# ecpoppenheimer/TensorFlowRayTrace

Measured on AMD Instinct MI355X. Metric: ray-surface intersection tests/sec (fwd+bwd), higher is better.
Workload: dtype f32 ray state, f32 filter + f64 decisions

## Files before the change

### tensorflowraytrace_amd/csrc/tfrt_trace3d.hip

```cpp
#include <vector>

#include <type_traits>
#include "tfrt_common.h"
#include "goal_finish.h"
#include "wave_schedule.h"

namespace tfrt {

constexpr int TILE = 512;
constexpr int KC = 24;

constexpr int ERR_CAPACITY = 1;


__global__ __launch_bounds__(BLOCK) void k_center(const double* __restrict__ fverts, int M,
                                                  double* __restrict__ c0, int32_t* nrays0, int n,
                                                  int32_t* tail8, unsigned int* scan_ticket) {
  if (nrays0 != nullptr) {
    if (threadIdx.x == 0) *nrays0 = n;
    if (threadIdx.x < 8) tail8[threadIdx.x] = 0;
    if (threadIdx.x == 0 && scan_ticket != nullptr) *scan_ticket = 0u;
  }
  __shared__ double red[WAVES][3];
  __shared__ double ctr[3];
// ... 1183 lines not shown
  float nx0, ny0, c0, nx1, ny1, c1, nx2, ny2, c2;
  edge(q0x, q0y, g1x, g1y, &nx0, &ny0, &c0);
  edge(q0x + g1x, q0y + g1y, g2x - g1x, g2y - g1y, &nx1, &ny1, &c1);
  edge(q0x + g2x, q0y + g2y, -g2x, -g2y, &nx2, &ny2, &c2);
  if (flat) {
    nx0 = ny0 = nx1 = ny1 = nx2 = ny2 = 0.f;
    c0 = c1 = c2 = -INFINITY;
  }
  const float slack2 = 1.5f * slack;
  rec[0] = make_float4(nx0, ny0, c0, tlo);
  rec[1] = make_float4(nx1, ny1, c1, thi);
  rec[2] = make_float4(nx2, ny2, c2, 0.5f * (tlo + thi));
  rec[3] = make_float4(0.5001f * (thi - tlo), slack2, r0.w, 0.f);
  const float rho = (fminf(b.R0 + b.S * fmaxf(fabsf(tlo), fabsf(thi)),
                           b.R0b + b.S * fmaxf(fabsf(tlo - b.tb), fabsf(thi - b.tb))) +
                     slack2) * 1.0001f;
  return !(c0 > rho) && !(c1 > rho) && !(c2 > rho) && !(thi < b.tmin);
}

template <typename Op>
__device__ __forceinline__ float wave_reduce_f(float v, Op op) {
  auto dpp = [](float x, auto ctrl, auto row_mask) {
    return __int_as_float(__builtin_amdgcn_update_dpp(__float_as_int(x), __float_as_int(x),
                                                      decltype(ctrl)::value,
                                                      decltype(row_mask)::value, 0xF, false));
  };
  using std::integral_constant;
  v = op(v, dpp(v, integral_constant<int, 0xB1>{}, integral_constant<int, 0xF>{}));
  v = op(v, dpp(v, integral_constant<int, 0x4E>{}, integral_constant<int, 0xF>{}));
  v = op(v, dpp(v, integral_constant<int, 0x141>{}, integral_constant<int, 0xF>{}));
  v = op(v, dpp(v, integral_constant<int, 0x140>{}, integral_constant<int, 0xF>{}));
  v = op(v, dpp(v, integral_constant<int, 0x142>{}, integral_constant<int, 0xA>{}));
  v = op(v, dpp(v, integral_constant<int, 0x143>{}, integral_constant<int, 0xC>{}));
  return __int_as_float(__builtin_amdgcn_readlane(__float_as_int(v), 63));
}
__device__ __forceinline__ float wave_sum_f(float v) {
  return wave_reduce_f(v, [](float a, float b) { return a + b; });
}
__device__ __forceinline__ float wave_max_f(float v) {
  return wave_reduce_f(v, [](float a, float b) { return fmaxf(a, b); });
}
__device__ __forceinline__ float wave_min_f(float v) {
  return wave_reduce_f(v, [](float a, float b) { return fminf(a, b); });
}
#define TFRT_DPP_STEP4(OPA, OPB, OPC, OPD, CTRL)      \
  OPA " %0, %0, %0 " CTRL "\n\t" OPB " %1, %1, %1 " CTRL "\n\t" \
  OPC " %2, %2, %2 " CTRL "\n\t" OPD " %3, %3, %3 " CTRL "\n\t"
#define TFRT_DPP_ALL4(OPA, OPB, OPC, OPD)                                        \
  "s_nop 1\n\t"                                                                  \
  TFRT_DPP_STEP4(OPA, OPB, OPC, OPD, "quad_perm:[1,0,3,2] row_mask:0xf bank_mask:0xf") \
  TFRT_DPP_STEP4(OPA, OPB, OPC, OPD, "quad_perm:[2,3,0,1] row_mask:0xf bank_mask:0xf") \
  TFRT_DPP_STEP4(OPA, OPB, OPC, OPD, "row_half_mirror row_mask:0xf bank_mask:0xf")     \
  TFRT_DPP_STEP4(OPA, OPB, OPC, OPD, "row_mirror row_mask:0xf bank_mask:0xf")          \
  TFRT_DPP_STEP4(OPA, OPB, OPC, OPD, "row_bcast:15 row_mask:0xa bank_mask:0xf")        \
  TFRT_DPP_STEP4(OPA, OPB, OPC, OPD, "row_bcast:31 row_mask:0xc bank_mask:0xf")
__device__ __forceinline__ void wave_sum4(float& a, float& b, float& c, float& d) {
  __asm__ volatile(TFRT_DPP_ALL4("v_add_f32_dpp", "v_add_f32_dpp", "v_add_f32_dpp", "v_add_f32_dpp")
                   : "+v"(a), "+v"(b), "+v"(c), "+v"(d));
  a = __int_as_float(__builtin_amdgcn_readlane(__float_as_int(a), 63));
  b = __int_as_float(__builtin_amdgcn_readlane(__float_as_int(b), 63));
  c = __int_as_float(__builtin_amdgcn_readlane(__float_as_int(c), 63));
  d = __int_as_float(__builtin_amdgcn_readlane(__float_as_int(d), 63));
}
__device__ __forceinline__ void wave_max3_min(float& a, float& b, float& c, float& d) {
  __asm__ volatile(TFRT_DPP_ALL4("v_max_f32_dpp", "v_max_f32_dpp", "v_max_f32_dpp", "v_min_f32_dpp")
                   : "+v"(a), "+v"(b), "+v"(c), "+v"(d));
  a = __int_as_float(__builtin_amdgcn_readlane(__float_as_int(a), 63));
  b = __int_as_float(__builtin_amdgcn_readlane(__float_as_int(b), 63));
  c = __int_as_float(__builtin_amdgcn_readlane(__float_as_int(c), 63));
  d = __int_as_float(__builtin_amdgcn_readlane(__float_as_int(d), 63));
}

#define TFRT_DPP_STEP3(OPA, OPB, OPC, CTRL) \
  OPA " %0, %0, %0 " CTRL "\n\t" OPB " %1, %1, %1 " CTRL "\n\t" OPC " %2, %2, %2 " CTRL "\n\t"
#define TFRT_DPP_ALL3(OPA, OPB, OPC)                                        \
  "s_nop 1\n\t"                                                             \
  TFRT_DPP_STEP3(OPA, OPB, OPC, "quad_perm:[1,0,3,2] row_mask:0xf bank_mask:0xf") \
  TFRT_DPP_STEP3(OPA, OPB, OPC, "quad_perm:[2,3,0,1] row_mask:0xf bank_mask:0xf") \
  TFRT_DPP_STEP3(OPA, OPB, OPC, "row_half_mirror row_mask:0xf bank_mask:0xf")     \
  TFRT_DPP_STEP3(OPA, OPB, OPC, "row_mirror row_mask:0xf bank_mask:0xf")          \
  TFRT_DPP_STEP3(OPA, OPB, OPC, "row_bcast:15 row_mask:0xa bank_mask:0xf")        \
  TFRT_DPP_STEP3(OPA, OPB, OPC, "row_bcast:31 row_mask:0xc bank_mask:0xf")
__device__ __forceinline__ void wave_sum2_max(float& a, float& b, float& c) {
  __asm__ volatile(TFRT_DPP_ALL3("v_add_f32_dpp", "v_add_f32_dpp", "v_max_f32_dpp")
                   : "+v"(a), "+v"(b), "+v"(c));
  a = __int_as_float(__builtin_amdgcn_readlane(__float_as_int(a), 63));
  b = __int_as_float(__builtin_amdgcn_readlane(__float_as_int(b), 63));
  c = __int_as_float(__builtin_amdgcn_readlane(__float_as_int(c), 63));
}

#define TFRT_BCAST(K) " row_newbcast:" #K " row_mask:0xf bank_mask:0xf\n\t"
__device__ __forceinline__ void face_edges(const float word, const float Ax, const float Ay,
                                           const float Mx, const float My, const float Mlen,
                                           const float Perr, const float Pm, float& room,
                                           float& e0, float& e1, float& e2) {
  float ix, iy;
  __asm__ volatile(
      "s_nop 1\n\t"
      "v_mov_b32_dpp %3, %6" TFRT_BCAST(11)
      "v_mov_b32_dpp %0, %6" TFRT_BCAST(13)
      "v_fma_f32 %5, %3, %10, %8\n\t"
      "v_fma_f32 %4, %3, %9, %7\n\t"
      "v_fmac_f32_dpp %0, %6, %11" TFRT_BCAST(12)
      "v_mul_f32_dpp %1, %6, %5" TFRT_BCAST(1)
      "v_mul_f32_dpp %2, %6, %5" TFRT_BCAST(5)
      "v_add_f32 %0, %12, %0\n\t"
      "v_fma_f32 %0, %13, |%3|, %0\n\t"
      "v_fmac_f32_dpp %1, %6, %4" TFRT_BCAST(0)
      "v_fmac_f32_dpp %2, %6, %4" TFRT_BCAST(4)
      "v_mul_f32_dpp %3, %6, %5" TFRT_BCAST(9)
      "v_add_f32_dpp %1, %6, %1" TFRT_BCAST(2)
      "v_add_f32_dpp %2, %6, %2" TFRT_BCAST(6)
      "v_fmac_f32_dpp %3, %6, %4" TFRT_BCAST(8)
      "s_nop 1\n\t"
      "v_add_f32_dpp %3, %6, %3" TFRT_BCAST(10)
      : "=&v"(room), "=&v"(e0), "=&v"(e1), "=&v"(e2), "=&v"(ix), "=&v"(iy)
      : "v"(word), "v"(Ax), "v"(Ay), "v"(Mx), "v"(My), "v"(Mlen), "v"(Perr), "v"(Pm));
}

__device__ __forceinline__ float uniform_f(float v) {
  return __int_as_float(__builtin_amdgcn_readfirstlane(__float_as_int(v)));
}
__device__ __forceinline__ float bcast_f(float v, int src_lane) {
  return __int_as_float(__builtin_amdgcn_readlane(__float_as_int(v), src_lane));
}

template <typename U>
using LdsPtr = __attribute__((address_space(3))) U*;

template <typename RT>
__device__ __forceinline__ void beam_decide(const int nb, const int lane, LdsPtr<const uint32_t> x_pair,
                                         LdsPtr<const RT> rt, LdsPtr<unsigned long long> best_k,
                                         LdsPtr<int32_t> best_i, const double* __restrict__ fverts,
                                         const double eps_int, const double eps_size,
                                         const double eps_start) {
  bool have = false;
  unsigned long long key = 0, old = 0;
  int j = -1;
  const uint32_t xp = lane < nb ? x_pair[lane] : 0u;
  const int slot = (int)(xp & 63u);
  if (lane < nb) {
    double s[3], e[3];
#pragma unroll
    for (int k = 0; k < 3; ++k) {
      s[k] = static_cast<double>(rt[k * 64 + slot]);
      e[k] = static_cast<double>(rt[(3 + k) * 64 + slot]);
    }
    j = (int)(xp >> 6);
    old = best_k[slot];
    double P[9];
    const double* fp = fverts + 9 * (int64_t)j;
#pragma unroll
    for (int k = 0; k < 9; ++k) P[k] = fp[k];
    const TriHit h = exact_triangle(s, e, P, eps_int, eps_size, eps_start);
    if (h.valid) {
      have = true;
      key = dkey(h.ray_u);
    }
  }
  wave_fence();
  if (have) atomicMin((unsigned long long*)&best_k[slot], key);
  wave_fence();
  bool win = false;
  if (have) {
    const unsigned long long now = best_k[slot];
    win = key == now;
    if (win && now < old) best_i[slot] = 0x7FFFFFFF;
  }
  wave_fence();
  if (win) atomicMin((int32_t*)&best_i[slot], j);
  wave_fence();
}

template <typename RT>
struct BeamLds {
  uint16_t slist[BEAM_SLIST];
  uint16_t clist[BEAM_CLIST];
  uint32_t flist[BEAM_FLIST];
  uint32_t x_pair[192];
  float4 ftab[65][4];
  RT rtab[6][64];
  unsigned long long best_k[64];
  int32_t best_i[64];
};

struct BeamScene {
  const float4* susphere;
  const float4* clsphere;
  const float4* csphere;
  const float4* crec;
  const double* fverts;
  const double* c0;
  int n_clusters, n_super;
  double eps_int, eps_size, eps_start;
};

#ifdef TFRT_TICKS
#define TFRT_WI_ARG _wi
#else
#define TFRT_WI_ARG nullptr
#endif

template <typename T, typename RT>
__device__ __forceinline__ bool beam_pass(BeamLds<RT>& W, const BeamScene& g, const int lane,
                                          const int bundle, const bool live, const int skip,
                                          const bool first_pass, const int coherent_only,
                                          unsigned* _wi, unsigned* work = nullptr) {
  TFRT_TICK_INIT;
  const float4* __restrict__ susphere = g.susphere;
  const float4* __restrict__ clsphere = g.clsphere;
  const float4* __restrict__ csphere = g.csphere;
  const float4* __restrict__ crec = g.crec;
  const double* __restrict__ fverts = g.fverts;
  const double* __restrict__ c0 = g.c0;
  const int n_clusters = g.n_clusters, n_super = g.n_super;
  const double eps_int = g.eps_int, eps_size = g.eps_size, eps_start = g.eps_start;
  const float4 never = make_float4(0.f, 0.f, 0.f, -1.f);
  W.best_k[lane] = dkey(INFINITY);
  W.best_i[lane] = -1;
  const double cx = c0[0], cy = c0[1], cz = c0[2];
  const float cxf = uniform_f((float)cx), cyf = uniform_f((float)cy), czf = uniform_f((float)cz);
  auto rel = [](const RT v, const double c, const float cf) -> float {
    if constexpr (sizeof(T) <= 4) return (float)v - cf;
    else return (float)((double)v - c);
  };
  const float es_f = (float)eps_size;
  int xn = 0;

  auto decide = [&](const int nb) {
    TFRT_STAT(28, 1);
    TFRT_WAVE_NOTE(1, 1);
    wave_fence();
    beam_decide<RT>(nb, lane, (LdsPtr<const uint32_t>)&W.x_pair[0],
                    (LdsPtr<const RT>)&W.rtab[0][0], (LdsPtr<unsigned long long>)&W.best_k[0],
                    (LdsPtr<int32_t>)&W.best_i[0], fverts, eps_int, eps_size, eps_start);
  };

  TFRT_STAT(8, 1);
  constexpr int BEAM_ATTEMPTS = 20;
  TFRT_TICK(0);
  float gap = -1.f;
  unsigned long long cuts = 0ull;
  int lo = 0, attempts = 0;
  bool spread = false;
  while (lo < bundle) {
    ++attempts;
    TFRT_STAT(30, 1);
    TFRT_WAVE_NOTE(0, 1);
    const unsigned long long above = lo < 63 ? (cuts >> (lo + 1)) << (lo + 1) : 0ull;
    const int hi = above != 0ull ? __ffsll((long long)above) - 1 : bundle;
    const int len = hi - lo;
    wave_fence();
    RT own[6];
#pragma unroll
    for (int k = 0; k < 6; ++k) own[k] = W.rtab[k][lane];
    const float sx = rel(own[0], cx, cxf), sy = rel(own[1], cy, cyf), sz = rel(own[2], cz, czf);
    const float dx = (float)(own[3] - own[0]), dy = (float)(own[4] - own[1]),
                dz = (float)(own[5] - own[2]);
    const float len2 = dx * dx + dy * dy + dz * dz;
    const bool ok = live && len2 > 0.f && len2 < 3.0e38f;
    const float inv = ok ? __builtin_amdgcn_rsqf(len2) : 0.f;
    const float ux = dx * inv, uy = dy * inv, uz = dz * inv;
    const float rabs = fabsf(sx) + fabsf(sy) + fabsf(sz);
    const bool sel = ok && lane >= lo && lane < hi;
    const float4 su_first = lane < n_super ? susphere[lane] : never;
    const float cnt = (float)__popcll(__ballot(sel));
    bool narrow = true, brute = false;
    int ns = 0, nc = 0, nf = 0;
    Beam bm = {0.f, 0.f, 0.f, 0.f, 0.f, 1.f, 0.f, 0.f, -INFINITY, 1.f, 0.f, 0.f, 0.f, 1.f, 0.f,
               INFINITY, 0.f};
    float ray_t = 0.f, ray_dt = 0.f, ray_terr = 0.f;
    float Ax = 0.f, Ay = 0.f, Mx = 0.f, My = 0.f, Mlen = 0.f, Perr = 0.f, Pm = 0.f;
    if (cnt > 0.f) {
      float swx = sel ? ux : 0.f, swy = sel ? uy : 0.f, swz = sel ? uz : 0.f;
      float sox = sel ? sx : 0.f, soy = sel ? sy : 0.f, soz = sel ? sz : 0.f;
      float Lw = sel ? rabs : 0.f;
      wave_sum4(swx, swy, swz, sox);
      wave_sum2_max(soy, soz, Lw);
      const float wl2 = swx * swx + swy * swy + swz * swz;
      narrow = wl2 > 0.49f * cnt * cnt;
      spread = !narrow;
      const float wi = narrow ? __builtin_amdgcn_rsqf(wl2) : 0.f;
      bm.wx = swx * wi; bm.wy = swy * wi; bm.wz = swz * wi;
      const float icnt = __builtin_amdgcn_rcpf(cnt);
      bm.ox = sox * icnt; bm.oy = soy * icnt; bm.oz = soz * icnt;
      const float cosk = ux * bm.wx + uy * bm.wy + uz * bm.wz;
      if (__any(sel && !(cosk > 0.7f))) narrow = false, spread = true;
      const float px = sx - bm.ox, py = sy - bm.oy, pz = sz - bm.oz;
      const float ts = px * bm.wx + py * bm.wy + pz * bm.wz;
      ray_t = ts;
      ray_dt = dx * bm.wx + dy * bm.wy + dz * bm.wz;
      ray_terr = 1e-5f * (rabs + fabsf(bm.ox) + fabsf(bm.oy) + fabsf(bm.oz));
      {
        const float f0 = fabsf(bm.wx), f1 = fabsf(bm.wy), f2 = fabsf(bm.wz);
        const bool k0 = f0 <= f1 && f0 <= f2, k1 = !k0 && f1 <= f2;
        const float kx = k0 ? 1.f : 0.f, ky = k1 ? 1.f : 0.f, kz = (!k0 && !k1) ? 1.f : 0.f;
        const float cxx = bm.wy * kz - bm.wz * ky, cyy = bm.wz * kx - bm.wx * kz,
                    czz = bm.wx * ky - bm.wy * kx;
        const float il = __builtin_amdgcn_rsqf(cxx * cxx + cyy * cyy + czz * czz);
        bm.e1x = cxx * il; bm.e1y = cyy * il; bm.e1z = czz * il;
        bm.e2x = bm.wy * bm.e1z - bm.wz * bm.e1y;
        bm.e2y = bm.wz * bm.e1x - bm.wx * bm.e1z;
        bm.e2z = bm.wx * bm.e1y - bm.wy * bm.e1x;
      }
      {
        const float idt = __builtin_amdgcn_rcpf(sel ? ray_dt : 1.f);
        Mx = (dx * bm.e1x + dy * bm.e1y + dz * bm.e1z) * idt;
        My = (dx * bm.e2x + dy * bm.e2y + dz * bm.e2z) * idt;
        const float p1 = px * bm.e1x + py * bm.e1y + pz * bm.e1z,
                    p2 = px * bm.e2x + py * bm.e2y + pz * bm.e2z;
        Ax = p1 - ts * Mx;
        Ay = p2 - ts * My;
        Mlen = __builtin_amdgcn_sqrtf(Mx * Mx + My * My) * 1.0001f;
        Pm = 2e-5f * (fabsf(Mx) + fabsf(My));
        Perr = 2e-5f * (fabsf(p1) + fabsf(p2) + fabsf(ts) * (fabsf(Mx) + fabsf(My)) + rabs +
                        fabsf(bm.ox) + fabsf(bm.oy) + fabsf(bm.oz));
      }
      float R0 = sel ? __builtin_amdgcn_sqrtf(Ax * Ax + Ay * Ay) : 0.f, S = sel ? Mlen : 0.f;
      float tmin = sel ? ts : INFINITY;
      Lw += fabsf(bm.ox) + fabsf(bm.oy) + fabsf(bm.oz);
      const float tb = -(bm.ox * bm.wx + bm.oy * bm.wy + bm.oz * bm.wz);
      float R0b = 0.f;
      if (sel) {
        const float bx = Ax + Mx * tb, by = Ay + My * tb;
        R0b = __builtin_amdgcn_sqrtf(bx * bx + by * by);
      }
      wave_max3_min(R0, S, R0b, tmin);
      bm.R0 = R0 * 1.001f + 4e-6f * Lw;
      bm.S = S * 1.001f + 2e-6f;
      bm.tb = tb;
      bm.R0b = R0b * 1.001f + 4e-6f * (Lw + fabsf(tb)) + 2e-6f * fabsf(tb) * S;
      if (!(bm.R0b < 3.0e38f)) bm.R0b = INFINITY;
      bm.tmin = (!first_pass && eps_start >= 0.0) ? tmin - 1e-5f * Lw - 1e-5f * fabsf(tmin)
                                                  : -INFINITY;
      if (!(bm.R0 < 3.0e38f && bm.S < 3.0e38f)) narrow = false;
      bm.ox = uniform_f(bm.ox); bm.oy = uniform_f(bm.oy); bm.oz = uniform_f(bm.oz);
      bm.wx = uniform_f(bm.wx); bm.wy = uniform_f(bm.wy); bm.wz = uniform_f(bm.wz);
      bm.R0 = uniform_f(bm.R0); bm.S = uniform_f(bm.S); bm.tmin = uniform_f(bm.tmin);
      bm.R0b = uniform_f(bm.R0b); bm.tb = uniform_f(bm.tb);
      bm.e1x = uniform_f(bm.e1x); bm.e1y = uniform_f(bm.e1y); bm.e1z = uniform_f(bm.e1z);
      bm.e2x = uniform_f(bm.e2x); bm.e2y = uniform_f(bm.e2y); bm.e2z = uniform_f(bm.e2z);
      TFRT_TICK(1);

      if (narrow) {
        float4 nxt = su_first;
        for (int b = 0; b < n_super; b += 64) {
          const int node = b + lane;
          const float4 cur = nxt;
          nxt = node + 64 < n_super ? susphere[node + 64] : never;
          const bool hit = beam_touch(bm, cur);
          const unsigned long long m = __ballot(hit);
          if (hit) {
            const int pos = ns + rank_below(m);
            if (pos < BEAM_SLIST) W.slist[pos] = (uint16_t)node;
          }
          ns += __popcll(m);
        }
        narrow = ns <= BEAM_SLIST && n_super <= 65536;
      }
      wave_fence();
      TFRT_TICK(2);
      if (narrow && ns > 0) {
        for (int b = 0; b < ns * SUPER; b += 64) {
          const int k = b + lane;
          bool hit = false;
          int cl = 0;
          if (k < ns * SUPER) {
            cl = (int)W.slist[k >> 3] * SUPER + (k & 7);
            if (cl < n_clusters) hit = beam_touch(bm, clsphere[cl]);
          }
          const unsigned long long m = __ballot(hit);
          if (hit) {
            const int pos = nc + rank_below(m);
            if (pos < BEAM_CLIST) W.clist[pos] = (uint16_t)cl;
// ... 55 lines not shown
      if (len == 1 && !hopeless) {
        brute = true;
      } else {
        TFRT_STAT(ns > BEAM_SLIST ? 10 : (nc > BEAM_CLIST ? 11 : (nf > BEAM_FLIST ? 12 : 9)), 1);
        TFRT_STAT(15, lo);
        return false;
      }
    }

    TFRT_STAT(13, nf);
    TFRT_WAVE_NOTE(3, nf);
    TFRT_TICK(5);
    auto reach_now = [&]() {
      const double best = dkey_inv(W.best_k[lane]);
      const float bu = next_up_f((float)best) * ray_dt;
      return ray_t + bu + 1e-5f * fabsf(bu) + ray_terr;
    };
    float myreach = reach_now();
    bool queued = false;
    const int n_cand = brute ? n_clusters * CLUSTER : nf;
    int f0 = 0;
    do {
      const int nb = min(64, n_cand - f0);
      if (work != nullptr) work[1] += (unsigned)nb;
      float4 rec[4] = {never, never, never, never};
      bool touch = false;
      float tnear = INFINITY;
      bool cand = lane < nb;
      if (brute && cand) {
        const float4 sp = csphere[f0 + lane];
        const float vx = sp.x - bm.ox, vy = sp.y - bm.oy, vz = sp.z - bm.oz;
        const float vu = vx * bm.wx + vy * bm.wy + vz * bm.wz;
        const float v2 = vx * vx + vy * vy + vz * vz;
        const float rr = __builtin_amdgcn_sqrtf(sp.w) * 1.000002f + bm.radius(vu, 0.f);
        cand = v2 - vu * vu <= rr * rr + 4e-6f * v2;
      }
      if (cand) {
        const int64_t memb = brute ? (int64_t)(f0 + lane) : (int64_t)W.flist[f0 + lane];
        const float4 r0 = crec[3 * memb], r1 = crec[3 * memb + 1], r2 = crec[3 * memb + 2];
        touch = face_frame(bm, r0, r1, r2, es_f, rec) && __float_as_int(r0.w) >= 0;
        tnear = rec[0].w;
        if (tnear != tnear) tnear = -INFINITY;
        rec[0].w = tnear;
      }
      f0 += 64;
      const bool closing = f0 >= n_cand && hi == bundle;
      const unsigned long long tm = __ballot(touch);
      const int nt = __popcll(tm);
      int place = 0;
      for (unsigned long long rest = tm; rest != 0ull; rest &= rest - 1ull) {
        const int o = __ffsll((long long)rest) - 1;
        const float to = bcast_f(tnear, o);
        place += (to < tnear || (to == tnear && o < lane)) ? 1 : 0;
      }
      wave_fence();
      if (touch) {
        W.ftab[place][0] = rec[0];
        W.ftab[place][1] = rec[1];
        W.ftab[place][2] = rec[2];
        W.ftab[place][3] = rec[3];
      }
      wave_fence();
      TFRT_STAT(27, nt);
      TFRT_TICK(6);
      float span = -INFINITY;
      auto on_face = [&](const float word, int* j, float* thi) {
        const float tn = bcast_f(word, 3);
        *thi = bcast_f(word, 7);
        *j = __float_as_int(bcast_f(word, 14));
        float room, e0, e1, e2;
        face_edges(word, Ax, Ay, Mx, My, Mlen, Perr, Pm, room, e0, e1, e2);
        const bool behind = bm.tmin > -INFINITY && *thi < ray_t - ray_terr;
        return (sel & (*j != skip) & !(myreach < tn) & !behind) &
               (!(e0 > room) & !(e1 > room) & !(e2 > room));
      };
      for (int c = 0;; c += 2) {
        const bool end = c >= nt;
        const bool two = c + 1 < nt;
        const float* recs = reinterpret_cast<const float*>(&W.ftab[end ? 0 : c][0]) + (lane & 15);
        const float word = recs[0], word2 = recs[16];
        const float tn = end ? INFINITY : bcast_f(word, 3);
        const bool flush =
            end ? closing
                : (tn > span && __ballot(sel && !(queued || myreach < INFINITY)) == 0ull);
        while (xn >= 64 || (flush && xn > 0)) {
          const int nd = min(xn, 64);
          wave_fence();
          decide(nd);
          uint32_t tp = 0u, tq = 0u;
          if (lane < xn - nd) tp = W.x_pair[nd + lane];
          if (lane + 64 < xn - nd) tq = W.x_pair[nd + 64 + lane];
          wave_fence();
          if (lane < xn - nd) W.x_pair[lane] = tp;
          if (lane + 64 < xn - nd) W.x_pair[64 + lane] = tq;
          xn -= nd;
          wave_fence();
          if (xn == 0) queued = false;
          myreach = reach_now();
          TFRT_TICK(8);
        }
        if (end) break;
        if (__ballot(sel && !(myreach < tn)) == 0ull) {
          c = nt - 2;
          continue;
        }
        TFRT_STAT(29, two ? 2 : 1);
        TFRT_WAVE_NOTE(2, two ? 2 : 1);
        int ja, jb = -1;
        float thia, thib = -INFINITY;
        const bool keepa = on_face(word, &ja, &thia);
        bool keepb = false;
        if (two) keepb = on_face(word2, &jb, &thib);
        span = fmaxf(span, fmaxf(thia, thib));
        const unsigned long long kma = __ballot(keepa), kmb = __ballot(keepb);
        const int na = __popcll(kma);
        if (keepa) W.x_pair[xn + rank_below(kma)] = ((uint32_t)ja << 6) | (uint32_t)lane;
        if (keepb) W.x_pair[xn + na + rank_below(kmb)] = ((uint32_t)jb << 6) | (uint32_t)lane;
        queued = queued || keepa || keepb;
        xn += na + __popcll(kmb);
        if (work != nullptr) work[0] += (unsigned)(na + __popcll(kmb));
        TFRT_STAT(14, na + __popcll(kmb));
        TFRT_TICK(7);
      }
    } while (f0 < n_cand);
    lo = hi;
  }
  wave_fence();
  return true;
}

template <typename T, int BW>
__global__ __launch_bounds__(64 * BW) void k_intersect_beam(
    const T* __restrict__ rays, int64_t stride, const int32_t* __restrict__ n_ptr,
    const int32_t* __restrict__ last_tri, BeamScene g, const int32_t* __restrict__ catagory,
    int32_t* __restrict__ rec_tri, double* __restrict__ rec_t, uint8_t* __restrict__ rec_cls,
    int32_t* __restrict__ hist, int32_t* __restrict__ left_list, int32_t* __restrict__ left_count,
    int32_t* __restrict__ left_total, int coherent_only, int bundle) {
  const int tid = threadIdx.x, lane = tid & 63, wave = tid >> 6;
  const int qwave = blockIdx.x * BW + wave;
  const int q = qwave * bundle + lane;
  const int n = *n_ptr;
  if (qwave * bundle >= n) return;
  TFRT_WAVE_BEGIN;

  using RT = std::conditional_t<sizeof(T) <= 4, float, double>;
  const int i = (lane < bundle && q < n) ? q : -1;
  const bool live = i >= 0;
  const int64_t ii = live ? i : 0;
  __shared__ BeamLds<RT> lds[BW];
  BeamLds<RT>& W = lds[wave];
#pragma unroll
  for (int k = 0; k < 6; ++k) W.rtab[k][lane] = static_cast<RT>(rays[k * stride + ii]);
  const int skip = (live && last_tri != nullptr) ? last_tri[ii] : -1;
  if (!beam_pass<T, RT>(W, g, lane, bundle, live, skip, last_tri == nullptr, coherent_only,
                        TFRT_WI_ARG)) {
    if (lane == 0) {
      left_list[atomicAdd(left_count, 1)] = qwave;
      atomicAdd(left_total, 1);
    }
    return;
  }
  wave_fence();

  int cls = -1;
  if (live) {
    const int bi = W.best_i[lane];
    cls = (bi < 0) ? CLS_DEAD : cat_to_cls(catagory[bi]);
    rec_tri[i] = bi;
    rec_t[i] = dkey_inv(W.best_k[lane]);
    rec_cls[i] = (uint8_t)cls;
  }
#pragma unroll
  for (int c = 0; c < 4; ++c) {
    const int cnt_c = __popcll(__ballot(cls == c));
    if (lane == c && cnt_c > 0) atomicAdd(&hist[((qwave * bundle) >> 8) * 4 + c], cnt_c);
  }
  TFRT_WAVE_END(qwave);
}


__global__ __launch_bounds__(BLOCK) void k_classify3d(
    const int32_t* __restrict__ n_ptr, int chunks, const double* __restrict__ part_t,
    const int32_t* __restrict__ part_i, int64_t part_stride,
    const int32_t* __restrict__ catagory, int32_t* __restrict__ rec_tri,
    double* __restrict__ rec_t, uint8_t* __restrict__ rec_cls, int32_t* __restrict__ blockcnt) {
  const int n = *n_ptr;
  const int base = blockIdx.x * BLOCK;
  if (base >= n) return;
  const int i = base + threadIdx.x;
  int cls = -1;
  if (i < n) {
    double bt = INFINITY;
    int bi = -1;
    for (int c = 0; c < chunks; ++c) {
      const double t = part_t[c * part_stride + i];
      const int pi = part_i[c * part_stride + i];
      if (t < bt || (t == bt && pi >= 0 && pi < bi)) {
        bt = t;
        bi = pi;
      }
    }
    cls = (bi < 0) ? CLS_DEAD : cat_to_cls(catagory[bi]);
    rec_tri[i] = bi;
    rec_t[i] = bt;
    rec_cls[i] = (uint8_t)cls;
  }
  __shared__ int wc[WAVES][4];
  const int wave = threadIdx.x >> 6;
#pragma unroll
  for (int c = 0; c < 4; ++c) {
    const unsigned long long m = __ballot(cls == c);
    if (lane_id() == 0) wc[wave][c] = __popcll(m);
  }
  __syncthreads();
  if (threadIdx.x < 4) {
    int s = 0;
    for (int w = 0; w < WAVES; ++w) s += wc[w][threadIdx.x];
    blockcnt[blockIdx.x * 4 + threadIdx.x] = s;
  }
}


__global__ __launch_bounds__(1024) void k_scan3d_one(const int32_t* __restrict__ n_ptr,
                                                 const int32_t* __restrict__ blockcnt,
                                                 int32_t* __restrict__ blockoff,
                                                 int32_t* __restrict__ pass_counts,
                                                 int32_t* __restrict__ totals,
                                                 int32_t* __restrict__ n_next,
                                                 unsigned long long* __restrict__ n_tests,
                                                 int M) {
  const int n = *n_ptr;
  const int nblk = (n + BLOCK - 1) / BLOCK;
  __shared__ int total[4];
  scan_rows_one<4>(blockcnt, blockoff, nblk, total);
  if (threadIdx.x < 4) {
    const int c = threadIdx.x;
    pass_counts[c] = total[c];
    pass_counts[4 + c] = totals[c];
    totals[c] += total[c];
  }
  if (threadIdx.x == 0) {
    *n_next = total[CLS_ACTIVE];
    *n_tests += (unsigned long long)n * (unsigned long long)M;
  }
}

constexpr int SCAN_GRID_MIN_ROWS = 8192;
__global__ __launch_bounds__(1024) void k_scan3d(const int32_t* __restrict__ n_ptr,
                                                 const int32_t* __restrict__ blockcnt,
                                                 int32_t* __restrict__ blockoff,
                                                 int32_t* __restrict__ rowtot,
                                                 int32_t* __restrict__ rowbase,
                                                 unsigned int* __restrict__ ticket,
                                                 int32_t* __restrict__ pass_counts,
                                                 int32_t* __restrict__ totals,
                                                 int32_t* __restrict__ n_next,
                                                 unsigned long long* __restrict__ n_tests,
                                                 int M) {
  const int n = *n_ptr;
  const int nblk = (n + BLOCK - 1) / BLOCK;
  __shared__ int total[4];
  if (!scan_rows_grid<4>(blockcnt, blockoff, nblk, rowtot, rowbase, ticket, total)) return;
  if (threadIdx.x < 4) {
    const int c = threadIdx.x;
    pass_counts[c] = total[c];
    pass_counts[4 + c] = totals[c];
    totals[c] += total[c];
  }
  if (threadIdx.x == 0) {
    *n_next = total[CLS_ACTIVE];
    *n_tests += (unsigned long long)n * (unsigned long long)M;
  }
}


__device__ __forceinline__ void face_indices(const tfrt_scene3d& sc, int tri, int rid,
                                             double* n_in, double* n_out) {
  if (sc.n_table != nullptr && sc.mat_in != nullptr) {
    const int64_t col = sc.n_table_uniform ? 0 : rid;
    *n_in = sc.n_table[(int64_t)sc.mat_in[tri] * sc.n_table_stride + col];
    *n_out = sc.n_table[(int64_t)sc.mat_out[tri] * sc.n_table_stride + col];
  } else {
    *n_in = sc.n_in[tri];
    *n_out = sc.n_out[tri];
  }
}

template <typename T>
__device__ __forceinline__ bool emit(const tfrt_ray_out& o, int64_t slot, const double s[3],
                                     const double e[3], int rid, int face) {
  if (o.rays == nullptr) return true;
  if (slot >= o.capacity) return false;
  store_ray3(static_cast<T*>(o.rays), o.capacity, slot, s, e);
  if (o.ray_id) o.ray_id[slot] = rid;
  if (o.face) o.face[slot] = face;
  return true;
}

constexpr int SELF_SCAN_MAX_BLOCKS = 4096;
struct SelfScan {
  const int32_t* blockcnt = nullptr;
  const int32_t* prev_counts = nullptr;
  int32_t* counts_row = nullptr;
  int32_t* totals = nullptr;
  int32_t* n_next = nullptr;
  unsigned long long* n_tests = nullptr;
  int M = 0;
  int32_t* hist_next = nullptr;
// ... 44 lines not shown
    const unsigned long long m = __ballot(cls == c);
    if (cls == c) rank = rank_below(m);
    if (lane_id() == 0) wc[wave][c] = __popcll(m);
  }
  if (self) {
    int loc[4] = {0, 0, 0, 0};
    const int4* __restrict__ rows = reinterpret_cast<const int4*>(ss.blockcnt);
    for (int b = threadIdx.x; b < (int)blockIdx.x; b += BLOCK) {
      const int4 v = rows[b];
      loc[0] += v.x;
      loc[1] += v.y;
      loc[2] += v.z;
      loc[3] += v.w;
    }
#pragma unroll
    for (int c = 0; c < 4; ++c) {
#pragma unroll
      for (int d = 32; d > 0; d >>= 1) loc[c] += __shfl_xor(loc[c], d, 64);
      if (lane_id() == 0) wpre[wave][c] = loc[c];
    }
  }
  __syncthreads();
  if (self && blockIdx.x == (unsigned)((n - 1) / BLOCK) && threadIdx.x < 4) {
    const int c = threadIdx.x;
    int total = 0;
    for (int w = 0; w < WAVES; ++w) total += wpre[w][c] + wc[w][c];
    ss.counts_row[c] = total;
    ss.counts_row[4 + c] = before[c];
    ss.totals[c] = before[c] + total;
    if (c == CLS_ACTIVE) *ss.n_next = total;
    if (c == 1) *ss.n_tests += (unsigned long long)n * (unsigned long long)ss.M;
  }
  if (i >= n) return;
  for (int w = 0; w < wave; ++w) rank += wc[w][cls];
  int slot;
  int64_t gslot;
  if (self) {
    int off = 0;
    for (int w = 0; w < WAVES; ++w) off += wpre[w][cls];
    slot = off + rank;
    gslot = (int64_t)before[cls] + slot;
  } else {
    slot = blockoff[blockIdx.x * 4 + cls] +
           (rowbase != nullptr ? rowbase[(blockIdx.x >> 10) * 4 + cls] : 0) + rank;
    gslot = (int64_t)pass_counts[4 + cls] + slot;
  }

  double s[3], e[3];
  load_ray3(rays_in, stride_in, i, s, e);
  const int rid = ray_id_in ? ray_id_in[i] : i;
  const int tri = rec_tri[i];
  bool ok = true;

  if (cls == CLS_DEAD) {
    if (flags & TFRT_COMPILE_DEAD) {
      double e2[3] = {e[0], e[1], e[2]};
      if (dead_len != 0.0)
        for (int k = 0; k < 3; ++k) e2[k] = advance_between(s[k], dead_len, e[k]);
      ok = emit<T>(dead, gslot, s, e2, rid, -1);
    }
    rec_slot[i] = (int32_t)gslot;
  } else {
    double h[3];
    hit_point(s, e, rec_t[i], h);
    if (cls == CLS_FINISHED) {
      if (flags & TFRT_COMPILE_FINISHED) ok = emit<T>(fin, gslot, s, h, rid, tri);
      rec_slot[i] = (int32_t)gslot;
    } else if (cls == CLS_STOPPED) {
      if (flags & TFRT_COMPILE_STOPPED) ok = emit<T>(stp, gslot, s, h, rid, tri);
      rec_slot[i] = (int32_t)gslot;
    } else {
      if (flags & TFRT_COMPILE_ACTIVE) ok = emit<T>(act, gslot, s, h, rid, tri);
      double un[3], n1, n2, n_in;
      const double* fp = fnorm + 3 * (int64_t)tri;
#pragma unroll
      for (int q = 0; q < 3; ++q) un[q] = fp[q];
      if (feta != nullptr) {
        const double* fe = feta + 4 * (int64_t)tri;
        n1 = fe[0];
        n2 = fe[1];
        n_in = fe[2];
      } else {
        double n_out;
        face_indices(sc, tri, rid, &n_in, &n_out);
        snell_ratios(n_in, n_out, &n1, &n2);
      }
      const Snell3 f = snell3d_core(s, h, un, n1, n2, n_in == 0.0);
      rec_cls[i] = (uint8_t)(cls | (f.nu > 0.0 ? TAPE_INTERNAL : 0) | (f.reflect ? TAPE_REFLECT : 0));
      double e2[3];
      for (int k = 0; k < 3; ++k) e2[k] = advance(h[k], L, f.w[k]);
      store_ray3(rays_out, stride_out, slot, h, e2);
      ray_id_out[slot] = rid;
      last_tri_out[slot] = tri;
      rec_slot[i] = slot;
      if (prep_next != nullptr) {
        double sr[3], er[3], u[3], scv[3];
        for (int k = 0; k < 3; ++k) {
          sr[k] = static_cast<double>(static_cast<T>(h[k]));
          er[k] = static_cast<double>(static_cast<T>(e2[k]));
        }
        float o[8];
        ray_filter_state(sr, er, c0, o, u, scv);
#pragma unroll
        for (int k = 0; k < 8; ++k) prep_next[k * pstride + slot] = o[k];
      }
    }
  }
  if (!ok) atomicOr(err, ERR_CAPACITY);
}

inline int inplace_bundle(int64_t N) { return N <= 160 * 1024 ? 32 : 64; }
inline size_t inplace_wstride(int64_t N) { return ((size_t)((N > 0 ? N : 1) + 31) / 32 + 63) / 64 * 64; }

template <typename T>
struct InplaceArgs {
  const T* src;
  int64_t src_stride;
  int32_t N, P, bundle, nwaves;
  const InplaceTape* tape;
  const int32_t* sched;
  int32_t ngroups, gshift;
};

#ifndef TFRT_INPLACE_WAVES
#define TFRT_INPLACE_WAVES 5
#endif
#define TFRT_INPLACE_ATTR __attribute__((amdgpu_waves_per_eu(TFRT_INPLACE_WAVES, TFRT_INPLACE_WAVES)))
template <typename T, bool ROWS>
__device__ __forceinline__ void trace_inplace(const InplaceArgs<T>& a, const BeamScene& g) {
  using RT = std::conditional_t<sizeof(T) <= 4, float, double>;
  const int lane = threadIdx.x;
  int qwave = blockIdx.x;
  if (a.sched != nullptr) {
    const int g = __builtin_amdgcn_readfirstlane(a.sched[blockIdx.x >> a.gshift]);
    if ((unsigned)g >= (unsigned)a.ngroups) return;
    qwave = (g << a.gshift) + ((int)blockIdx.x & ((1 << a.gshift) - 1));
    if (qwave >= a.nwaves) return;
  }
  const int q = qwave * a.bundle + lane;
  const bool has = lane < a.bundle && q < a.N;
  const int64_t i = has ? q : 0;
  __shared__ BeamLds<RT> lds;
  BeamLds<RT>& W = lds;
#pragma unroll
  for (int k = 0; k < 6; ++k) W.rtab[k][lane] = static_cast<RT>(a.src[k * a.src_stride + i]);
  bool active = has;
  int skip = -1;
  int p = 0;
  static_assert(sizeof(InplaceTape) % 4 == 0 && sizeof(InplaceTape) / 4 <= 64, "one word per lane");
  const uint32_t tape_words =
      reinterpret_cast<const uint32_t*>(a.tape)[lane < (int)(sizeof(InplaceTape) / 4) ? lane : 0];
  TFRT_WAVE_BEGIN;
  unsigned work[2] = {0u, 0u};
  for (; p < a.P; ++p) {
    if (__ballot(active) == 0ull) break;
    beam_pass<T, RT>(W, g, lane, a.bundle, active, skip, p == 0, 1, TFRT_WI_ARG,
                     work);
    wave_fence();
    TFRT_TICK_INIT;
    uint32_t tw = tape_words;
    __asm__ volatile("" : "+v"(tw));
    InplaceTape tq;
    {
      uint32_t w[sizeof(InplaceTape) / 4];
#pragma unroll
      for (int k = 0; k < (int)(sizeof(InplaceTape) / 4); ++k)
        w[k] = (uint32_t)__builtin_amdgcn_readlane((int)tw, k);
      __builtin_memcpy(&tq, w, sizeof(InplaceTape));
    }
    int cls = -1;
    if (active) {
      const int bi = W.best_i[lane];
      const double t = dkey_inv(W.best_k[lane]);
      cls = (bi < 0) ? CLS_DEAD : cat_to_cls(tq.catagory[bi]);
      const size_t at = (size_t)p * tq.n + i;
      tq.rec_tri[at] = bi;
      tq.rec_t[at] = t;
      int tape = cls;
      if (cls == CLS_ACTIVE) {
        double s[3], e[3], h[3];
#pragma unroll
        for (int k = 0; k < 3; ++k) {
          s[k] = static_cast<double>(W.rtab[k][lane]);
          e[k] = static_cast<double>(W.rtab[3 + k][lane]);
        }
        hit_point(s, e, t, h);
        double un[3], n1, n2, n_in;
        const double* fp = tq.fnorm + 3 * (int64_t)bi;
#pragma unroll
        for (int k = 0; k < 3; ++k) un[k] = fp[k];
        if (tq.feta != nullptr) {
          const double* fe = tq.feta + 4 * (int64_t)bi;
          n1 = fe[0];
          n2 = fe[1];
          n_in = fe[2];
        } else {
          n_in = tq.n_table[(int64_t)tq.mat_in[bi] * tq.n_table_stride + i];
          const double n_out = tq.n_table[(int64_t)tq.mat_out[bi] * tq.n_table_stride + i];
          snell_ratios(n_in, n_out, &n1, &n2);
        }
        const Snell3 f = snell3d_core(s, h, un, n1, n2, n_in == 0.0);
        tape |= (f.nu > 0.0 ? TAPE_INTERNAL : 0) | (f.reflect ? TAPE_REFLECT : 0);
        T* out = static_cast<T*>(tq.rays_ws) + (size_t)p * 6 * tq.n;
#pragma unroll
        for (int k = 0; k < 3; ++k) {
          const T hs = static_cast<T>(h[k]);
          const T es = static_cast<T>(advance(h[k], tq.L, f.w[k]));
          out[k * tq.n + i] = hs;
          out[(3 + k) * tq.n + i] = es;
          W.rtab[k][lane] = static_cast<RT>(hs);
          W.rtab[3 + k][lane] = static_cast<RT>(es);
        }
        skip = bi;
      } else {
        active = false;
        if (ROWS) {
          const bool fin = cls == CLS_FINISHED;
          T* fin_rows = static_cast<T*>(tq.fin_rows);
          double h[3] = {0.0, 0.0, 0.0};
          if (fin) {
            double s[3], e[3];
#pragma unroll
            for (int k = 0; k < 3; ++k) {
              s[k] = static_cast<double>(W.rtab[k][lane]);
              e[k] = static_cast<double>(W.rtab[3 + k][lane]);
            }
            hit_point(s, e, t, h);
          }
#pragma unroll
          for (int k = 0; k < 3; ++k) {
            fin_rows[k * tq.fin_cap + i] = fin ? static_cast<T>(W.rtab[k][lane]) : a.src[k * a.src_stride + i];
            fin_rows[(3 + k) * tq.fin_cap + i] = fin ? static_cast<T>(h[k]) : a.src[(3 + k) * a.src_stride + i];
          }
          tq.fin_face[i] = fin ? bi : -1;
          tq.fin_passes[i] = p + 1;
        }
      }
      tq.rec_cls[at] = (uint8_t)tape;
    }
    uint32_t word = 0u;
#pragma unroll
    for (int c = 0; c < 4; ++c) word |= (uint32_t)__popcll(__ballot(cls == c)) << (8 * c);
    if (lane == 0) tq.wcount[(size_t)p * tq.wstride + qwave] = word;
    TFRT_TICK(11);
  }
  InplaceTape te;
  {
    uint32_t w[sizeof(InplaceTape) / 4];
#pragma unroll
    for (int k = 0; k < (int)(sizeof(InplaceTape) / 4); ++k)
      w[k] = (uint32_t)__builtin_amdgcn_readlane((int)tape_words, k);
    __builtin_memcpy(&te, w, sizeof(InplaceTape));
  }
  if (ROWS && active) {
    T* fin_rows = static_cast<T*>(te.fin_rows);
#pragma unroll
    for (int k = 0; k < 6; ++k) fin_rows[k * te.fin_cap + i] = a.src[k * a.src_stride + i];
    te.fin_face[i] = -1;
    te.fin_passes[i] = a.P;
  }
  for (int pp = p + lane; pp < a.P; pp += 64) te.wcount[(size_t)pp * te.wstride + qwave] = 0u;
  if (lane < 2) te.wcount[(size_t)(a.P + lane) * te.wstride + qwave] = work[lane];
  TFRT_WAVE_END(qwave);
}

template <typename T>
__global__ __launch_bounds__(64) TFRT_INPLACE_ATTR void k_trace_inplace(InplaceArgs<T> a, BeamScene g) {
  trace_inplace<T, false>(a, g);
}
template <typename T>
__global__ __launch_bounds__(64) __attribute__((amdgpu_waves_per_eu(4, 4))) void k_trace_inplace_rows(
    InplaceArgs<T> a, BeamScene g) {
  trace_inplace<T, true>(a, g);
}

__global__ __launch_bounds__(1024) void k_inplace_scan(const uint32_t* __restrict__ wcount,
                                                       int nwaves, int wstride, int P, int N, int M,
                                                       int4* __restrict__ wbase,
                                                       int32_t* __restrict__ counts) {
  const int p = blockIdx.x, tid = threadIdx.x, lane = tid & 63, wave = tid >> 6;
  __shared__ int wsum[16][4];
  __shared__ int red[4];
  auto unpack = [](uint32_t w, int v[4]) {
#pragma unroll
    for (int c = 0; c < 4; ++c) v[c] += (int)((w >> (8 * c)) & 0xFFu);
  };
  int before[4] = {0, 0, 0, 0};
  if (p > 0) {
    int acc[4] = {0, 0, 0, 0};
    for (int q = 0; q < p; ++q) {
      const uint32_t* rq = wcount + (size_t)q * wstride;
      for (int k0 = tid; k0 < nwaves; k0 += 8 * 1024) {
        uint32_t w[8];
#pragma unroll
        for (int j = 0; j < 8; ++j) w[j] = (k0 + j * 1024 < nwaves) ? rq[k0 + j * 1024] : 0u;
#pragma unroll
        for (int j = 0; j < 8; ++j) unpack(w[j], acc);
      }
    }
#pragma unroll
    for (int c = 0; c < 4; ++c) {
#pragma unroll
      for (int d = 32; d > 0; d >>= 1) acc[c] += __shfl_xor(acc[c], d, 64);
      if (lane == 0) wsum[wave][c] = acc[c];
    }
    __syncthreads();
    if (tid < 4) {
      int r = 0;
      for (int w = 0; w < 16; ++w) r += wsum[w][tid];
      red[tid] = r;
    }
    __syncthreads();
#pragma unroll
    for (int c = 0; c < 4; ++c) before[c] = red[c];
    __syncthreads();
  }
  const uint4* row4 = reinterpret_cast<const uint4*>(wcount + (size_t)p * wstride);
  int4* out = wbase + (size_t)p * wstride;
  int tot[4] = {0, 0, 0, 0};
  for (int base = 0; base < nwaves; base += 16 * 1024) {
    const int w0 = base + tid * 16;
    uint32_t w[16];
#pragma unroll
    for (int j = 0; j < 4; ++j) {
      const uint4 v = (w0 + 4 * j < nwaves) ? row4[(w0 >> 2) + j] : make_uint4(0u, 0u, 0u, 0u);
      w[4 * j] = v.x;
      w[4 * j + 1] = v.y;
      w[4 * j + 2] = v.z;
      w[4 * j + 3] = v.w;
    }
    int mine[4] = {0, 0, 0, 0};
#pragma unroll
    for (int j = 0; j < 16; ++j) {
      if (w0 + j >= nwaves) w[j] = 0u;
      unpack(w[j], mine);
    }
    int pre[4];
#pragma unroll
    for (int c = 0; c < 4; ++c) {
      int x = mine[c];
#pragma unroll
      for (int d = 1; d < 64; d <<= 1) {
        const int o = __shfl_up(x, d, 64);
        if (lane >= d) x += o;
      }
// ... 2151 lines not shown
```

### tensorflowraytrace_amd/csrc/trace_math.h

```cpp
#pragma once
#include <math.h>

#if defined(__HIPCC__)
#define TFRT_HD __host__ __device__ __forceinline__
#else
#define TFRT_HD inline
#endif

namespace tfrt {

constexpr int CLS_ACTIVE = 0;
constexpr int CLS_FINISHED = 1;
constexpr int CLS_STOPPED = 2;
constexpr int CLS_DEAD = 3;

constexpr int CAT_OPTICAL = 0, CAT_STOP = 1, CAT_TARGET = 2;

struct TriHit {
  double ray_u, trig_u, trig_v;
  bool valid;
};

TFRT_HD TriHit exact_triangle(const double s[3], const double e[3], const double P[9],
                              double eps_int, double eps_size, double eps_start) {
#pragma clang fp contract(off)
  const double a = s[0] - e[0], d = s[1] - e[1], h = s[2] - e[2];
  const double b = P[3] - P[0], f = P[4] - P[1], k = P[5] - P[2];
  const double c = P[6] - P[0], g = P[7] - P[1], l = P[8] - P[2];
  const double q = s[0] - P[0], r = s[1] - P[1], t = s[2] - P[2];

  const double den = a * g * k + b * d * l + c * f * h - a * f * l - b * g * h - c * d * k;
  const double nr = b * l * r + c * f * t + g * k * q - b * g * t - c * k * r - f * l * q;
  const double nu = a * g * t + c * h * r + d * l * q - a * l * r - c * d * t - g * h * q;
  const double nv = a * k * r + b * d * t + f * h * q - a * f * t - b * h * r - d * k * q;

  TriHit o;
  bool valid = fabs(den) >= eps_int;
  const double sd = valid ? den : 1.0;
  o.ray_u = nr / sd;
  o.trig_u = nu / sd;
  o.trig_v = nv / sd;
  valid = valid && (o.trig_u >= -eps_size);
  valid = valid && (o.trig_v >= -eps_size);
  valid = valid && (o.trig_u + o.trig_v <= 1.0 + eps_size);
  valid = valid && (o.ray_u >= eps_start);
  o.valid = valid;
  return o;
}

TFRT_HD float next_up_f(float x) {
  x += 0.0f;
  unsigned b;
  __builtin_memcpy(&b, &x, 4);
  const unsigned up = b + (unsigned)(((int)b >> 31) | 1);
  float y;
  __builtin_memcpy(&y, &up, 4);
  return x < INFINITY ? y : x;
}

TFRT_HD void hit_point(const double s[3], const double e[3], double ray_u, double h[3]) {
#pragma clang fp contract(off)
  h[0] = s[0] - ray_u * (s[0] - e[0]);
  h[1] = s[1] - ray_u * (s[1] - e[1]);
  h[2] = s[2] - ray_u * (s[2] - e[2]);
}

TFRT_HD double advance(double origin, double L, double dir) {
#pragma clang fp contract(off)
  return origin + L * dir;
}

TFRT_HD double advance_between(double s, double L, double e) {
#pragma clang fp contract(off)
  return s + L * (e - s);
}

TFRT_HD void cross3(const double a[3], const double b[3], double o[3]) {
#pragma clang fp contract(off)
  o[0] = a[1] * b[2] - a[2] * b[1];
  o[1] = a[2] * b[0] - a[0] * b[2];
  o[2] = a[0] * b[1] - a[1] * b[0];
}

TFRT_HD double dot3(const double a[3], const double b[3]) {
#pragma clang fp contract(off)
  return a[0] * b[0] + a[1] * b[1] + a[2] * b[2];
}

TFRT_HD void face_normal(const double P[9], double N[3], double C[3], double* clen) {
#pragma clang fp contract(off)
  const double A[3] = {P[3] - P[0], P[4] - P[1], P[5] - P[2]};
  const double B[3] = {P[6] - P[3], P[7] - P[4], P[8] - P[5]};
  cross3(A, B, C);
  const double len = sqrt(dot3(C, C));
  *clen = len;
  N[0] = C[0] / len;
  N[1] = C[1] / len;
  N[2] = C[2] / len;
}

TFRT_HD double l2_normalize3(const double v[3], double o[3]) {
#pragma clang fp contract(off)
  double sq = dot3(v, v);
  if (sq < 1e-12) sq = 1e-12;
  const double inv = 1.0 / sqrt(sq);
  o[0] = v[0] * inv;
  o[1] = v[1] * inv;
  o[2] = v[2] * inv;
  return inv;
}

struct Snell3 {
  double u[3], n[3];
  double nu, eta, k;
  bool reflect;
  double w[3];
};

TFRT_HD void snell_normal(const double P[9], double n[3]) {
  double N[3], C[3], clen;
  face_normal(P, N, C, &clen);
  l2_normalize3(N, n);
}

TFRT_HD void snell_ratios(double n_in, double n_out, double* n1, double* n2) {
#pragma clang fp contract(off)
  const bool in_safe = n_in != 0.0, out_safe = n_out != 0.0;
  const double nis = in_safe ? n_in : 1.0, nos = out_safe ? n_out : 1.0;
  *n1 = out_safe ? nis / nos : 0.0;
  *n2 = in_safe ? nos / nis : 0.0;
}

TFRT_HD Snell3 snell3d_core(const double s[3], const double h[3], const double un[3], double n1,
                            double n2, bool mirror) {
#pragma clang fp contract(off)
  Snell3 o;
  const double r[3] = {h[0] - s[0], h[1] - s[1], h[2] - s[2]};
  l2_normalize3(r, o.u);
  o.n[0] = un[0];
  o.n[1] = un[1];
  o.n[2] = un[2];
  o.nu = dot3(o.n, o.u);
  const bool internal = o.nu > 0.0;
  o.eta = internal ? n1 : n2;
  const double nu_eta = o.eta * o.nu;
  o.k = 1.0 - o.eta * o.eta + nu_eta * nu_eta;
  const bool tir = o.k < 0.0;
  o.reflect = tir || mirror;
  if (o.reflect) {
    for (int i = 0; i < 3; ++i) o.w[i] = -2.0 * o.nu * o.n[i] + o.u[i];
  } else {
    const double sg = (o.nu > 0.0) ? 1.0 : ((o.nu < 0.0) ? -1.0 : 0.0);
    const double alpha = sg * sqrt(o.k) - nu_eta;
    for (int i = 0; i < 3; ++i) o.w[i] = alpha * o.n[i] + o.eta * o.u[i];
  }
  return o;
}

TFRT_HD Snell3 snell3d_unit(const double s[3], const double h[3], const double un[3],
                            double n_in, double n_out) {
  double n1, n2;
  snell_ratios(n_in, n_out, &n1, &n2);
  return snell3d_core(s, h, un, n1, n2, n_in == 0.0);
}

TFRT_HD Snell3 snell3d(const double s[3], const double h[3], const double norm[3],
                       double n_in, double n_out) {
  double un[3];
  l2_normalize3(norm, un);
  return snell3d_unit(s, h, un, n_in, n_out);
}

TFRT_HD double fmod_floor(double x, double m) {
  double r = fmod(x, m);
  if (r != 0.0 && ((r < 0.0) != (m < 0.0))) r += m;
  return r;
}

TFRT_HD double snell2d_angle(double xs, double ys, double xe, double ye, double norm,
                             double n_in, double n_out) {
#pragma clang fp contract(off)
  const double PI = 3.141592653589793;
  norm = fmod_floor(norm, 2 * PI);
  double ray_angle = atan2(ys - ye, xs - xe);
  ray_angle = fmod_floor(ray_angle, 2 * PI);
  double theta1 = norm - ray_angle;
  if (theta1 > PI) theta1 = theta1 - 2 * PI;
  if (theta1 < -PI) theta1 = theta1 + 2 * PI;
  const bool internal = fabs(theta1) >= PI / 2;
  const bool in_safe = n_in != 0.0, out_safe = n_out != 0.0;
  const double nis = in_safe ? n_in : 1.0, nos = out_safe ? n_out : 1.0;
  const double n1 = out_safe ? nis / nos : 0.0;
  const double n2 = in_safe ? nos / nis : 0.0;
  const double n = internal ? n1 : n2;
// ... 195 lines not shown
```

Baseline: 139600 billion.

## Share f64 reciprocal across triangle quotients, hoist beam centre and face loads

Adds quotients3, which computes the three f64 divisions by the same denominator from one shared reciprocal refinement (div_scale/rcp/fma/div_fixup) when the scaled denominators match, and otherwise falls back to plain division. It is used only in beam_decide's exact triangle test. The beam centre (c0 and its float copy) is now loaded once per kernel and passed into beam_pass instead of being reloaded each pass. In the in-place tracer, the face normal, category and eta loads are issued together before classification so their latencies overlap. The shared-reciprocal path must stay bit-identical to IEEE division, which the div_fixup sequence is meant to guarantee.

```diff
diff --git a/tensorflowraytrace_amd/csrc/tfrt_trace3d.hip b/tensorflowraytrace_amd/csrc/tfrt_trace3d.hip
--- a/tensorflowraytrace_amd/csrc/tfrt_trace3d.hip
+++ b/tensorflowraytrace_amd/csrc/tfrt_trace3d.hip
@@ -1359,7 +1359,7 @@
     const double* fp = fverts + 9 * (int64_t)j;
 #pragma unroll
     for (int k = 0; k < 9; ++k) P[k] = fp[k];
-    const TriHit h = exact_triangle(s, e, P, eps_int, eps_size, eps_start);
+    const TriHit h = exact_triangle<true>(s, e, P, eps_int, eps_size, eps_start);
     if (h.valid) {
       have = true;
       key = dkey(h.ray_u);
@@ -1408,8 +1408,23 @@
 #define TFRT_WI_ARG nullptr
 #endif
 
+struct BeamCentre {
+  double c[3];
+  float cf[3];
+};
+__device__ __forceinline__ BeamCentre beam_centre(const double* __restrict__ c0) {
+  BeamCentre o;
+#pragma unroll
+  for (int k = 0; k < 3; ++k) {
+    o.c[k] = c0[k];
+    o.cf[k] = uniform_f((float)o.c[k]);
+  }
+  return o;
+}
+
 template <typename T, typename RT>
-__device__ __forceinline__ bool beam_pass(BeamLds<RT>& W, const BeamScene& g, const int lane,
+__device__ __forceinline__ bool beam_pass(BeamLds<RT>& W, const BeamScene& g,
+                                          const BeamCentre& ctr, const int lane,
                                           const int bundle, const bool live, const int skip,
                                           const bool first_pass, const int coherent_only,
                                           unsigned* _wi, unsigned* work = nullptr) {
@@ -1419,14 +1434,13 @@
   const float4* __restrict__ csphere = g.csphere;
   const float4* __restrict__ crec = g.crec;
   const double* __restrict__ fverts = g.fverts;
-  const double* __restrict__ c0 = g.c0;
   const int n_clusters = g.n_clusters, n_super = g.n_super;
   const double eps_int = g.eps_int, eps_size = g.eps_size, eps_start = g.eps_start;
   const float4 never = make_float4(0.f, 0.f, 0.f, -1.f);
   W.best_k[lane] = dkey(INFINITY);
   W.best_i[lane] = -1;
-  const double cx = c0[0], cy = c0[1], cz = c0[2];
-  const float cxf = uniform_f((float)cx), cyf = uniform_f((float)cy), czf = uniform_f((float)cz);
+  const double cx = ctr.c[0], cy = ctr.c[1], cz = ctr.c[2];
+  const float cxf = ctr.cf[0], cyf = ctr.cf[1], czf = ctr.cf[2];
   auto rel = [](const RT v, const double c, const float cf) -> float {
     if constexpr (sizeof(T) <= 4) return (float)v - cf;
     else return (float)((double)v - c);
@@ -1788,8 +1802,8 @@
 #pragma unroll
   for (int k = 0; k < 6; ++k) W.rtab[k][lane] = static_cast<RT>(rays[k * stride + ii]);
   const int skip = (live && last_tri != nullptr) ? last_tri[ii] : -1;
-  if (!beam_pass<T, RT>(W, g, lane, bundle, live, skip, last_tri == nullptr, coherent_only,
-                        TFRT_WI_ARG)) {
+  if (!beam_pass<T, RT>(W, g, beam_centre(g.c0), lane, bundle, live, skip, last_tri == nullptr,
+                        coherent_only, TFRT_WI_ARG)) {
     if (lane == 0) {
       left_list[atomicAdd(left_count, 1)] = qwave;
       atomicAdd(left_total, 1);
@@ -2140,10 +2154,11 @@
       reinterpret_cast<const uint32_t*>(a.tape)[lane < (int)(sizeof(InplaceTape) / 4) ? lane : 0];
   TFRT_WAVE_BEGIN;
   unsigned work[2] = {0u, 0u};
+  const BeamCentre centre = beam_centre(g.c0);
   for (; p < a.P; ++p) {
     if (__ballot(active) == 0ull) break;
-    beam_pass<T, RT>(W, g, lane, a.bundle, active, skip, p == 0, 1, TFRT_WI_ARG,
-                     work);
+    beam_pass<T, RT>(W, g, centre, lane, a.bundle, active, skip, p == 0, 1,
+                     TFRT_WI_ARG, work);
     wave_fence();
     TFRT_TICK_INIT;
     uint32_t tw = tape_words;
@@ -2160,7 +2175,20 @@
     if (active) {
       const int bi = W.best_i[lane];
       const double t = dkey_inv(W.best_k[lane]);
-      cls = (bi < 0) ? CLS_DEAD : cat_to_cls(tq.catagory[bi]);
+      int cat = 0;
+      double un[3] = {0.0, 0.0, 0.0}, fe[3] = {0.0, 0.0, 0.0};
+      if (bi >= 0) {
+        cat = tq.catagory[bi];
+        const double* fp = tq.fnorm + 3 * (int64_t)bi;
+#pragma unroll
+        for (int k = 0; k < 3; ++k) un[k] = fp[k];
+        if (tq.feta != nullptr) {
+          const double* fq = tq.feta + 4 * (int64_t)bi;
+#pragma unroll
+          for (int k = 0; k < 3; ++k) fe[k] = fq[k];
+        }
+      }
+      cls = (bi < 0) ? CLS_DEAD : cat_to_cls(cat);
       const size_t at = (size_t)p * tq.n + i;
       tq.rec_tri[at] = bi;
       tq.rec_t[at] = t;
@@ -2173,12 +2201,8 @@
           e[k] = static_cast<double>(W.rtab[3 + k][lane]);
         }
         hit_point(s, e, t, h);
-        double un[3], n1, n2, n_in;
-        const double* fp = tq.fnorm + 3 * (int64_t)bi;
-#pragma unroll
-        for (int k = 0; k < 3; ++k) un[k] = fp[k];
+        double n1, n2, n_in;
         if (tq.feta != nullptr) {
-          const double* fe = tq.feta + 4 * (int64_t)bi;
           n1 = fe[0];
           n2 = fe[1];
           n_in = fe[2];
diff --git a/tensorflowraytrace_amd/csrc/trace_math.h b/tensorflowraytrace_amd/csrc/trace_math.h
--- a/tensorflowraytrace_amd/csrc/trace_math.h
+++ b/tensorflowraytrace_amd/csrc/trace_math.h
@@ -21,6 +21,42 @@
   bool valid;
 };
 
+TFRT_HD void quotients3(double nr, double nu, double nv, double sd, double* qr, double* qu,
+                        double* qv) {
+#pragma clang fp contract(off)
+#if defined(__HIP_DEVICE_COMPILE__)
+  bool fr, fu, fv;
+  const double dr = __builtin_amdgcn_div_scale(nr, sd, false, &fr);
+  const double du = __builtin_amdgcn_div_scale(nu, sd, false, &fu);
+  const double dv = __builtin_amdgcn_div_scale(nv, sd, false, &fv);
+  unsigned long long br, bu, bv;
+  __builtin_memcpy(&br, &dr, 8);
+  __builtin_memcpy(&bu, &du, 8);
+  __builtin_memcpy(&bv, &dv, 8);
+  if ((br == bu) & (br == bv)) {
+    const double nd = -dr;
+    const double r0 = __builtin_amdgcn_rcp(dr);
+    const double r1 = __builtin_fma(r0, __builtin_fma(nd, r0, 1.0), r0);
+    const double r2 = __builtin_fma(r1, __builtin_fma(nd, r1, 1.0), r1);
+    const double num[3] = {nr, nu, nv};
+    double* const out[3] = {qr, qu, qv};
+#pragma unroll
+    for (int k = 0; k < 3; ++k) {
+      bool fn;
+      const double ns = __builtin_amdgcn_div_scale(num[k], sd, true, &fn);
+      const double m = ns * r2;
+      const double res = __builtin_fma(nd, m, ns);
+      *out[k] = __builtin_amdgcn_div_fixup(__builtin_amdgcn_div_fmas(res, r2, m, fn), sd, num[k]);
+    }
+    return;
+  }
+#endif
+  *qr = nr / sd;
+  *qu = nu / sd;
+  *qv = nv / sd;
+}
+
+template <bool SHARED_QUOTIENTS = false>
 TFRT_HD TriHit exact_triangle(const double s[3], const double e[3], const double P[9],
                               double eps_int, double eps_size, double eps_start) {
 #pragma clang fp contract(off)
@@ -37,9 +73,13 @@
   TriHit o;
   bool valid = fabs(den) >= eps_int;
   const double sd = valid ? den : 1.0;
-  o.ray_u = nr / sd;
-  o.trig_u = nu / sd;
-  o.trig_v = nv / sd;
+  if constexpr (SHARED_QUOTIENTS) {
+    quotients3(nr, nu, nv, sd, &o.ray_u, &o.trig_u, &o.trig_v);
+  } else {
+    o.ray_u = nr / sd;
+    o.trig_u = nu / sd;
+    o.trig_v = nv / sd;
+  }
   valid = valid && (o.trig_u >= -eps_size);
   valid = valid && (o.trig_v >= -eps_size);
   valid = valid && (o.trig_u + o.trig_v <= 1.0 + eps_size);
```

After: 141400 billion (median of 6 runs). +1.3%, better.
